# HITRainer/EAVSR

Measured on AMD Instinct MI355X. Metric: SR frames/sec at 4x 7-frame 180x320->720x1280, higher is better.
Workload: dtype f32

## Files before the change

### eavsr_amd/csrc/conv_x6.hip

```cpp
#include "common.h"

#include <mutex>

namespace {

typedef const __attribute__((address_space(1))) void* gptr_t;
typedef __attribute__((address_space(3))) void* lptr_t;
typedef unsigned u32x4 __attribute__((ext_vector_type(4)));
typedef __bf16 bf16x8 __attribute__((ext_vector_type(8)));

constexpr int S_NW = 8, S_TW = 32;
template <int KS, int MT, int NT, int NP = 3> struct C7 {
  static constexpr int PAD = KS / 2, KK = KS * KS;
  static constexpr int KSTEPS = (KK + 1) / 2;
  static constexpr int SLAB = KS == 5 ? 7 : 5;
  static constexpr int NSLAB = (KSTEPS + SLAB - 1) / SLAB;
  static constexpr int TH = S_NW * NT;
  static constexpr int IH = TH + KS - 1;
  static constexpr int IW = S_TW + KS;
  static constexpr int NPIX = IH * IW;
  static constexpr int PLANE_B = NPIX * 16;
  static constexpr int PATCH_B = NP * PLANE_B;
  static constexpr int KS_U4 = NP * MT * 64;
  static constexpr int SLAB_U4 = SLAB * KS_U4;
  static constexpr size_t LDS_BYTES = 2 * (size_t)PATCH_B + 2 * (size_t)SLAB_U4 * 16 + 64 * 4;
  static_assert(NPIX <= 1024, "two patch pixels per thread");
  static_assert(LDS_BYTES <= 160 * 1024, "LDS");
};

struct C7Args {
  const float* x;
  const u32x4* wsplit;
  const float* bias;
  float* out;
  int n, cin, cout, h, w, tiles_x, tiles_y;
  int act;
  float slope;
  int sig_from;
};

__device__ __forceinline__ void s_split2(float a, float b, unsigned& hi, unsigned& mid, unsigned& lo) {
  const unsigned ua = __float_as_uint(a), ub = __float_as_uint(b);
  const float ra = a - __uint_as_float(ua & 0xFFFF0000u), rb = b - __uint_as_float(ub & 0xFFFF0000u);
  const unsigned uma = __float_as_uint(ra), umb = __float_as_uint(rb);
  const float la = ra - __uint_as_float(uma & 0xFFFF0000u), lb = rb - __uint_as_float(umb & 0xFFFF0000u);
  hi = __builtin_amdgcn_perm(ub, ua, 0x07060302u);
  mid = __builtin_amdgcn_perm(umb, uma, 0x07060302u);
  lo = __builtin_amdgcn_perm(__float_as_uint(lb), __float_as_uint(la), 0x07060302u);
}

__device__ __forceinline__ f32x16 s_mfma(const u32x4& a, const u32x4& b, const f32x16& c) {
  return __builtin_amdgcn_mfma_f32_32x32x16_bf16(__builtin_bit_cast(bf16x8, a), __builtin_bit_cast(bf16x8, b), c, 0, 0, 0);
}
typedef _Float16 s_h16x8 __attribute__((ext_vector_type(8)));
__device__ __forceinline__ f32x16 s_mfma_f16(const u32x4& a, const u32x4& b, const f32x16& c) {
  return __builtin_amdgcn_mfma_f32_32x32x16_f16(__builtin_bit_cast(s_h16x8, a), __builtin_bit_cast(s_h16x8, b), c, 0, 0, 0);
}
template <int DT> __device__ __forceinline__ unsigned s_round2(float a, float b) {
  if (DT == 1) return (unsigned)__builtin_bit_cast(unsigned short, (_Float16)a) | ((unsigned)__builtin_bit_cast(unsigned short, (_Float16)b) << 16);
  typedef float f2_ __attribute__((ext_vector_type(2)));
  typedef __bf16 b2_ __attribute__((ext_vector_type(2)));
  return __builtin_bit_cast(unsigned, __builtin_convertvector(f2_{a, b}, b2_));
}

#ifdef EAVSR_C7_STAMPS
__device__ unsigned long long g_c7_stamps[8];
#define C7_STAMP(i)                                                   \
  do {                                                                \
    const unsigned long long t_ = __builtin_amdgcn_s_memtime();       \
    st_acc[i] += t_ - st_last;                                        \
    st_last = t_;                                                     \
  } while (0)
#else
#define C7_STAMP(i) do { } while (0)
#endif

template <int KS, int MT, int NT, int WMT, int NP = 3, int DT = 0, bool PERSIST = false>
__global__ __launch_bounds__(512) void conv_x6_kernel(C7Args a) {
  static_assert((NP == 3 && DT == 0) || (NP == 1 && (DT == 1 || DT == 2)), "three exact bf16 planes, or one rounded fp16 / bf16 plane");
  using K = C7<KS, MT, NT, NP>;
  constexpr int S_NT = NT, S_TH = K::TH, S_NPIX = K::NPIX, S_PLANE_B = K::PLANE_B, S_PATCH_B = K::PATCH_B;
  constexpr int S_PAD = K::PAD, S_IW = K::IW, S_KSTEPS = K::KSTEPS, S_SLAB = K::SLAB, S_NSLAB = K::NSLAB;
#ifdef EAVSR_C7_STAMPS
  unsigned long long st_acc[8] = {0, 0, 0, 0, 0, 0, 0, 0};
  unsigned long long st_last = __builtin_amdgcn_s_memtime();
#endif
  extern __shared__ __attribute__((aligned(16))) unsigned char smem7[];
  unsigned char* s_patch = smem7;
  u32x4* s_w = reinterpret_cast<u32x4*>(smem7 + 2 * S_PATCH_B);
  float* s_bias = reinterpret_cast<float*>(smem7 + 2 * S_PATCH_B + 2 * K::SLAB_U4 * 16);

  const int tid = threadIdx.x;
  const int lane = tid & 63;
  const int wave = __builtin_amdgcn_readfirstlane(tid >> 6);
#if defined(EAVSR_X6_PRIO) && EAVSR_X6_PRIO == 1
  if (wave < 4) __builtin_amdgcn_s_setprio(1);
#elif defined(EAVSR_X6_PRIO) && EAVSR_X6_PRIO == 2
  if (wave >= 4) __builtin_amdgcn_s_setprio(1);
#endif
  const int l31 = lane & 31, kg = lane >> 5;

  const int ntiles = a.tiles_x * a.tiles_y * a.n;
  int tile = PERSIST ? (int)blockIdx.x : eavsr_xcd_remap(blockIdx.x, gridDim.x);
  int bn, y0, x0;
  auto place = [&](int t_, int& bn_, int& y0_, int& x0_) __attribute__((always_inline)) {
    const int tx = t_ % a.tiles_x;
    t_ /= a.tiles_x;
    bn_ = t_ / a.tiles_y;
    y0_ = (t_ - bn_ * a.tiles_y) * S_TH;
    x0_ = tx * S_TW;
  };
  place(tile, bn, y0, x0);
  const int cot = blockIdx.y;
  const int h = a.h, w = a.w;
  const size_t plane = (size_t)h * w;
  const int nch = a.cin >> 3;

  bool pok[2];
  unsigned pgo[2], plo[2];
  int pbn;
  auto aim_patch = [&](int t_) __attribute__((always_inline)) {
    int py0, px0;
    place(t_, pbn, py0, px0);
#pragma unroll
    for (int i = 0; i < 2; ++i) {
      const int p = tid + i * 512;
      const int r = p / S_IW, c = p - r * S_IW;
      const int gy = py0 - S_PAD + r, gx = px0 - S_PAD + c;
      pok[i] = p < S_NPIX && c < S_IW - 1 && gy >= 0 && gy < h && gx >= 0 && gx < w;
      pgo[i] = pok[i] ? (unsigned)(gy * w + gx) : 0u;
      plo[i] = (unsigned)p * 16u;
    }
  };
  aim_patch(tile);
  const bool second = tid + 512 < S_NPIX;
  float pv[2][8];
  auto load_patch = [&](int ch) __attribute__((always_inline)) {
    const float* sp = a.x + ((size_t)pbn * a.cin + (size_t)ch * 8) * plane;
#pragma unroll
    for (int i = 0; i < 2; ++i)
#pragma unroll
      for (int j = 0; j < 8; ++j) pv[i][j] = pok[i] ? sp[(size_t)j * plane + pgo[i]] : 0.f;
  };
  auto store_patch = [&](int stage) __attribute__((always_inline)) {
#pragma unroll
    for (int i = 0; i < 2; ++i) {
      if (i == 0 ? tid >= S_NPIX : !second) break;
      u32x4 pl[NP];
#pragma unroll
      for (int c = 0; c < 4; ++c) {
        if constexpr (NP == 3) {
          unsigned h2, m2, l2;
          s_split2(pv[i][2 * c], pv[i][2 * c + 1], h2, m2, l2);
          pl[0][c] = h2; pl[1][c] = m2; pl[2][c] = l2;
        } else {
          pl[0][c] = s_round2<DT>(pv[i][2 * c], pv[i][2 * c + 1]);
        }
      }
#pragma unroll
      for (int p3 = 0; p3 < NP; ++p3)
        *reinterpret_cast<u32x4*>(s_patch + stage * S_PATCH_B + p3 * S_PLANE_B + plo[i]) = pl[p3];
    }
  };
  const int nslabs = nch * S_NSLAB;
  constexpr int wsplit_n = WMT / MT;
  const int wcot = cot / wsplit_n, wsub = (cot - wcot * wsplit_n) * MT;
  auto issue_slab = [&](int gs, int ch, int si) __attribute__((always_inline)) {
    const int nks = (si + 1) * S_SLAB <= S_KSTEPS ? S_SLAB : S_KSTEPS - si * S_SLAB;
    const int segs = nks * NP * MT;
    const char* wsrc = reinterpret_cast<const char*>(a.wsplit + (((size_t)wcot * nch + ch) * S_KSTEPS + si * S_SLAB) * (K::KS_U4 * wsplit_n));
    u32x4* dst = s_w + (gs & 1) * K::SLAB_U4;
#pragma unroll
    for (int i = 0; i < (S_SLAB * NP * MT + S_NW - 1) / S_NW; ++i) {
      const int seg = i * S_NW + wave;
      if (seg < segs) {
        const int sp = MT == 1 ? seg * WMT + wsub : (seg >> 1) * WMT + wsub + (seg & 1);
        __builtin_amdgcn_global_load_lds((gptr_t)(wsrc + (unsigned)(sp * 64 + lane) * 16u), (lptr_t)(dst + seg * 64), 16, 0, 0);
      }
    }
  };

  f32x16 acc[MT][S_NT];

  const int bbase = ((wave * S_NT) * S_IW + l31) * 16;
  const int b_same = bbase + (kg ? 16 : 0);
  const int b_wrap = bbase + (kg ? (S_IW - (KS - 1)) * 16 : 0);
  const int b_last = kg ? (S_IW - 1) * 16 - ((KS - 1) * S_IW + KS - 1) * 16 : bbase;
  auto read_b = [&](int stage, int s, u32x4 (&b)[S_NT][NP]) __attribute__((always_inline)) {
    const int tap0 = 2 * s, ky = tap0 / KS, kx = tap0 - KS * ky;
    const unsigned char* base = s_patch + stage * S_PATCH_B + ((s == S_KSTEPS - 1 ? b_last : kx == KS - 1 ? b_wrap : b_same) + (ky * S_IW + kx) * 16);
#pragma unroll
    for (int t = 0; t < S_NT; ++t)
#pragma unroll
      for (int p3 = 0; p3 < NP; ++p3) b[t][p3] = *reinterpret_cast<const u32x4*>(base + t * S_IW * 16 + p3 * S_PLANE_B);
  };
  auto read_a = [&](int gs, int sl, u32x4 (&av)[NP][MT]) __attribute__((always_inline)) {
    const u32x4* ws = s_w + (gs & 1) * K::SLAB_U4 + sl * K::KS_U4 + lane;
#pragma unroll
    for (int p3 = 0; p3 < NP; ++p3)
#pragma unroll
      for (int m = 0; m < MT; ++m) av[p3][m] = ws[(p3 * MT + m) * 64];
  };

  issue_slab(0, 0, 0);
  load_patch(0);
  if (tid < 32 * MT) {
    const int co = cot * 32 * MT + tid;
    s_bias[tid] = (a.bias && co < a.cout) ? a.bias[co] : 0.f;
  }
  store_patch(0);
  asm volatile("s_waitcnt vmcnt(0)" ::: "memory");
  __syncthreads();
  auto init_acc = [&]() __attribute__((always_inline)) {
#pragma unroll
    for (int m = 0; m < MT; ++m)
#pragma unroll
      for (int r = 0; r < 16; ++r) {
        const float bv = s_bias[m * 32 + (r & 3) + 8 * (r >> 2) + 4 * kg];
#pragma unroll
        for (int t = 0; t < S_NT; ++t) acc[m][t][r] = bv;
      }
  };
  init_acc();
  if (nslabs > 1) issue_slab(1, S_NSLAB > 1 ? 0 : 1, S_NSLAB > 1 ? 1 : 0);
  u32x4 acur[NP][MT], bcur[S_NT][NP];
  read_a(0, 0, acur);
  read_b(0, 0, bcur);
  C7_STAMP(0);

  for (;;) {
  const bool has_next = PERSIST && tile + (int)gridDim.x < ntiles;
  for (int ch = 0; ch < nch; ++ch) {
    const int pst = ch & 1;
    const bool last_ch = ch + 1 == nch;
    const bool more = !last_ch || has_next;
    if (!last_ch) load_patch(ch + 1);
    else if (has_next) {
      aim_patch(tile + (int)gridDim.x);
      load_patch(0);
    }
#pragma unroll
    for (int ks = 0; ks < S_KSTEPS; ++ks) {
      constexpr int STORE_KS = KS == 7 ? 11 : KS == 5 ? 7 : 3;
      const int si = ks / S_SLAB, sl = ks % S_SLAB;
      const int gs = ch * S_NSLAB + si;
      const bool slab_end = sl == S_SLAB - 1 || ks == S_KSTEPS - 1;
      if (slab_end) {
        C7_STAMP(1);
        asm volatile("s_waitcnt vmcnt(0)" ::: "memory");
        C7_STAMP(2);
        __syncthreads();
        C7_STAMP(3);
        if (gs + 2 < nslabs) issue_slab(gs + 2, ch + (si + 2) / S_NSLAB, (si + 2) % S_NSLAB);
        else if (has_next) issue_slab(gs + 2 - nslabs, (gs + 2 - nslabs) / S_NSLAB, (si + 2) % S_NSLAB);
        C7_STAMP(4);
      }
      if (ks == STORE_KS && more) store_patch(pst ^ 1);
      u32x4 anext[NP][MT], bnext[S_NT][NP];
      const bool last = ks == S_KSTEPS - 1;
      if (!last) {
        read_a(slab_end ? gs + 1 : gs, slab_end ? 0 : sl + 1, anext);
        read_b(pst, ks + 1, bnext);
      } else if (more) {
        read_a(gs + 1, 0, anext);
        read_b(pst ^ 1, 0, bnext);
      }
#pragma unroll
      for (int t = 0; t < S_NT; ++t)
#pragma unroll
        for (int m = 0; m < MT; ++m) {
          f32x16 c_ = acc[m][t];
          if constexpr (NP == 3) {
            c_ = s_mfma(acur[2][m], bcur[t][0], c_);
            c_ = s_mfma(acur[0][m], bcur[t][2], c_);
            c_ = s_mfma(acur[1][m], bcur[t][1], c_);
            c_ = s_mfma(acur[1][m], bcur[t][0], c_);
            c_ = s_mfma(acur[0][m], bcur[t][1], c_);
            c_ = s_mfma(acur[0][m], bcur[t][0], c_);
          } else if constexpr (DT == 1) {
            c_ = s_mfma_f16(acur[0][m], bcur[t][0], c_);
          } else {
            c_ = s_mfma(acur[0][m], bcur[t][0], c_);
          }
          acc[m][t] = c_;
        }
      {
        constexpr int NRD = NP * MT + NP * S_NT, NMF = (NP == 3 ? 6 : 1) * MT * S_NT;
        constexpr int NIL = NRD < NMF ? NRD : NMF;
#pragma unroll
        for (int i = 0; i < NIL; ++i) {
          __builtin_amdgcn_sched_group_barrier(0x008, 1, 0);
          __builtin_amdgcn_sched_group_barrier(0x100, 1, 0);
        }
        if constexpr (NMF > NRD) __builtin_amdgcn_sched_group_barrier(0x008, NMF - NRD, 0);
        if constexpr (NRD > NMF) __builtin_amdgcn_sched_group_barrier(0x100, NRD - NMF, 0);
        __builtin_amdgcn_sched_barrier(0);
      }
      if (!last || more) {
#pragma unroll
        for (int p3 = 0; p3 < NP; ++p3) {
#pragma unroll
          for (int m = 0; m < MT; ++m) acur[p3][m] = anext[p3][m];
#pragma unroll
          for (int t = 0; t < S_NT; ++t) bcur[t][p3] = bnext[t][p3];
        }
      }
    }
  }

  C7_STAMP(1);
  {
  int gx = x0 + l31;
  asm volatile("" : "+v"(gx));
  const bool xok = gx < w;
  const float act_s = a.act == EAVSR_ACT_NONE ? 1.f : a.act == EAVSR_ACT_RELU ? 0.f : a.slope;
  const int co0 = cot * 32 * MT + 4 * kg;
  float* ob = a.out + ((size_t)bn * a.cout + co0) * plane + (size_t)(y0 + wave * S_NT) * w + gx;
  const bool full = cot * 32 * MT + 32 * MT <= a.cout;
#pragma unroll
  for (int m = 0; m < MT; ++m)
#pragma unroll
    for (int r = 0; r < 16; ++r) {
      const int cu = m * 32 + (r & 3) + 8 * (r >> 2);
      const bool cok = full || co0 + cu < a.cout;
      const bool sg = a.sig_from >= 0 && cot * 32 * MT + m * 32 + 8 * (r >> 2) >= a.sig_from;
#pragma unroll
      for (int t = 0; t < S_NT; ++t) {
        float v = acc[m][t][r];
        if (sg) v = eavsr_sigmoid_fast(v);
        else v = eavsr_act(v, act_s);
        if (cok && xok && y0 + wave * S_NT + t < h) ob[(size_t)cu * plane + (size_t)t * w] = v;
      }
    }
  }
  if (!has_next) break;
  tile += (int)gridDim.x;
  place(tile, bn, y0, x0);
  init_acc();
  }
#ifdef EAVSR_C7_STAMPS
  C7_STAMP(5);
  asm volatile("s_waitcnt vmcnt(0)" ::: "memory");
  C7_STAMP(6);
  if (tid == 0)
    for (int i = 0; i < 8; ++i) atomicAdd(&g_c7_stamps[i], st_acc[i]);
#endif
}

__global__ void pack7_kernel(const float* __restrict__ wt, u32x4* __restrict__ p, int cout, int cin, int kk, int mt_n, long total,
                             int np = 3, int dt = 0, int tr = 0) {
  const int ksteps = (kk + 1) / 2;
  const long e = (long)blockIdx.x * blockDim.x + threadIdx.x;
  if (e >= total) return;
  long q = e;
  const int lane = (int)(q % 64); q /= 64;
  const int mt = (int)(q % mt_n); q /= mt_n;
  const int pl = (int)(q % np); q /= np;
  const int s = (int)(q % ksteps); q /= ksteps;
  const int nch = cin / 8;
  const int ch = (int)(q % nch);
  const int cot = (int)(q / nch);
  const int co = cot * 32 * mt_n + mt * 32 + (lane & 31);
  const int tap = 2 * s + (lane >> 5);
  u32x4 o;
#pragma unroll
  for (int c = 0; c < 4; ++c) {
    float v[2];
#pragma unroll
    for (int u = 0; u < 2; ++u) {
      const int ci = ch * 8 + 2 * c + u;
      v[u] = (co < cout && tap < kk) ? (tr ? wt[((size_t)ci * cout + co) * kk + (kk - 1 - tap)] : wt[((size_t)co * cin + ci) * kk + tap]) : 0.f;
    }
    if (np == 3) {
      unsigned h2, m2, l2;
      s_split2(v[0], v[1], h2, m2, l2);
      o[c] = pl == 0 ? h2 : pl == 1 ? m2 : l2;
    } else {
      o[c] = dt == 1 ? s_round2<1>(v[0], v[1]) : s_round2<2>(v[0], v[1]);
    }
  }
  p[e] = o;
}

constexpr int PM_MAX = 48;
struct PackMultiArgs {
  const float* src[PM_MAX];
  u32x4* dst[PM_MAX];
  unsigned long long tr_mask;
};
template <int NP>
__global__ void pack7_multi_kernel(PackMultiArgs a, int cout, int cin, int kk, int mt_n, long total) {
  const int t = blockIdx.y;
  const int tr = (int)((a.tr_mask >> t) & 1ull);
  const float* __restrict__ wt = a.src[t];
  u32x4* __restrict__ p = a.dst[t];
  const int ksteps = (kk + 1) / 2;
  const long e = (long)blockIdx.x * blockDim.x + threadIdx.x;
  if (e >= total) return;
  long q = e;
  const int lane = (int)(q % 64); q /= 64;
  const int mt = (int)(q % mt_n); q /= mt_n;
  const int pl = (int)(q % NP); q /= NP;
  const int s = (int)(q % ksteps); q /= ksteps;
  const int nch = cin / 8;
  const int ch = (int)(q % nch);
  const int cot = (int)(q / nch);
  const int co = cot * 32 * mt_n + mt * 32 + (lane & 31);
  const int tap = 2 * s + (lane >> 5);
  u32x4 o;
#pragma unroll
  for (int c = 0; c < 4; ++c) {
    float v[2];
#pragma unroll
    for (int u = 0; u < 2; ++u) {
      const int ci = ch * 8 + 2 * c + u;
      v[u] = (co < cout && tap < kk) ? (tr ? wt[((size_t)ci * cout + co) * kk + (kk - 1 - tap)] : wt[((size_t)co * cin + ci) * kk + tap]) : 0.f;
    }
    if constexpr (NP == 3) {
      unsigned h2, m2, l2;
      s_split2(v[0], v[1], h2, m2, l2);
      o[c] = pl == 0 ? h2 : pl == 1 ? m2 : l2;
    } else {
      o[c] = s_round2<2>(v[0], v[1]);
    }
  }
  p[e] = o;
}

int mt_of(int cout) { return cout > 32 ? 2 : 1; }

int cu_count() {
  static int cus_pd[eavsr::kMaxDevices] = {};
  static eavsr::PerDeviceOnce once_pd;
  const int dev_ = eavsr::current_device();
  std::call_once(once_pd.flag[dev_], [&] {
    int v = 0;
    if (hipDeviceGetAttribute(&v, hipDeviceAttributeMultiprocessorCount, dev_) == hipSuccess && v > 0) cus_pd[dev_] = v;
  });
  return cus_pd[dev_];
}

int persist_grid(long tiles, int cot_n, int cin) {
  const int slots = cu_count() / cot_n;
  if (slots < 1 || tiles <= slots || (cin >> 3) % 2) return 0;
  const long rounds = (tiles + slots - 1) / slots;
  return (int)((tiles + rounds - 1) / rounds);
}

template <int KS, int MT, int NT, int WMT, int NP = 3, int DT = 0, bool PERSIST = false>
int launch7(const C7Args& a, void* stream, int grid_x = 0) {
  using K = C7<KS, MT, NT, NP>;
  static_assert(!PERSIST || K::NSLAB % 2 == 0, "the slab ring must come round to stage 0 at a tile's start");
  static eavsr::PerDeviceOnce once_pd;
  const int dev_ = eavsr::current_device();
  static hipError_t attr_err_pd[eavsr::kMaxDevices] = {};
  hipError_t& attr_err = attr_err_pd[dev_];
  std::call_once(once_pd.flag[dev_], [&] {
    attr_err = hipFuncSetAttribute(reinterpret_cast<const void*>(&conv_x6_kernel<KS, MT, NT, WMT, NP, DT, PERSIST>),
                                   hipFuncAttributeMaxDynamicSharedMemorySize, (int)K::LDS_BYTES);
  });
  if (attr_err != hipSuccess) {
    eavsr::set_error("conv_f32x6: hipFuncSetAttribute(%zu B of LDS): %s", K::LDS_BYTES, hipGetErrorString(attr_err));
    return (int)attr_err;
  }
  C7Args b = a;
  b.tiles_y = eavsr::cdiv(a.h, K::TH);
  const long blocks = (long)b.tiles_x * b.tiles_y * b.n;
  EAVSR_REQUIRE(blocks < (1L << 31), -1, "conv_f32x6: too many tiles");
  dim3 grid((unsigned)(PERSIST ? grid_x : blocks), eavsr::cdiv(a.cout, 32 * MT));
  hipLaunchKernelGGL((conv_x6_kernel<KS, MT, NT, WMT, NP, DT, PERSIST>), grid, dim3(64 * S_NW), K::LDS_BYTES, eavsr::as_stream(stream), b);
  return eavsr::launch_status("conv_f32x6");
}

template <int KS, int NP = 3, int DT = 0>
int dispatch7(const C7Args& a, void* stream) {
  const long wg2 = (long)a.tiles_x * eavsr::cdiv(a.h, 16) * a.n;
  const long wg1 = (long)a.tiles_x * eavsr::cdiv(a.h, 8) * a.n;
  EAVSR_REQUIRE(wg1 * 2 < (1L << 31), -1, "conv_f32x6: too many tiles");
  if (mt_of(a.cout) == 2) {
    if constexpr (KS == 5 && NP == 3) {
      const int g = wg2 >= 128 ? persist_grid(wg2, eavsr::cdiv(a.cout, 64), a.cin) : 0;
      if (g > 0) return launch7<KS, 2, 2, 2, NP, DT, true>(a, stream, g);
    }
    if (wg2 >= 128) return launch7<KS, 2, 2, 2, NP, DT>(a, stream);
    if (wg1 >= 128) return launch7<KS, 2, 1, 2, NP, DT>(a, stream);
    return launch7<KS, 1, 1, 2, NP, DT>(a, stream);
  }
  if (wg2 >= 128) return launch7<KS, 1, 2, 1, NP, DT>(a, stream);
  return launch7<KS, 1, 1, 1, NP, DT>(a, stream);
}

}

#ifdef EAVSR_C7_STAMPS
extern "C" int eavsr_debug_c7_stamps(unsigned long long* host_out, int reset) {
  hipError_t e = hipMemcpyFromSymbol(host_out, HIP_SYMBOL(g_c7_stamps), sizeof(unsigned long long) * 8);
  if (e != hipSuccess) return (int)e;
  if (reset) {
    unsigned long long z[8] = {0, 0, 0, 0, 0, 0, 0, 0};
    e = hipMemcpyToSymbol(HIP_SYMBOL(g_c7_stamps), z, sizeof(z));
  }
  return (int)e;
}
#endif

extern "C" size_t eavsr_conv_weight_x6_bytes(int32_t ksize, int32_t cout, int32_t cin) {
  if ((ksize != 3 && ksize != 5 && ksize != 7) || cout <= 0 || cin <= 0 || cin % 8) return 0;
  const int mt = mt_of(cout);
  return (size_t)eavsr::cdiv(cout, 32 * mt) * (cin / 8) * ((ksize * ksize + 1) / 2) * 3 * mt * 64 * 16;
}

extern "C" int eavsr_pack_conv_weight_x6(const float* weight, void* packed, int32_t ksize, int32_t cout, int32_t cin, void* stream) {
  EAVSR_REQUIRE(weight && packed, -1, "pack_conv_weight_x6: NULL pointer");
  EAVSR_REQUIRE(ksize == 3 || ksize == 5 || ksize == 7, -2, "pack_conv_weight_x6: kernel size %d (3, 5 and 7 only)", ksize);
  EAVSR_REQUIRE(cout > 0 && cin > 0 && cin % 8 == 0, -1, "pack_conv_weight_x6: cin %d must be a multiple of 8", cin);
  const long total = (long)(eavsr_conv_weight_x6_bytes(ksize, cout, cin) / 16);
  hipLaunchKernelGGL(pack7_kernel, dim3((unsigned)((total + 255) / 256)), dim3(256), 0, eavsr::as_stream(stream), weight,
                     reinterpret_cast<u32x4*>(packed), cout, cin, ksize * ksize, mt_of(cout), total);
  return eavsr::launch_status("pack_conv_weight_x6");
}

extern "C" int eavsr_pack_conv_weight_x6_dgrad(const float* weight, void* packed, int32_t ksize, int32_t cout_w, int32_t cin_w, void* stream) {
  EAVSR_REQUIRE(weight && packed, -1, "pack_conv_weight_x6_dgrad: NULL pointer");
  EAVSR_REQUIRE(ksize == 3 || ksize == 5 || ksize == 7, -2, "pack_conv_weight_x6_dgrad: kernel size %d (3, 5 and 7 only)", ksize);
  EAVSR_REQUIRE(cout_w > 0 && cin_w > 0 && cout_w % 8 == 0, -1, "pack_conv_weight_x6_dgrad: cout %d must be a multiple of 8", cout_w);
  const long total = (long)(eavsr_conv_weight_x6_bytes(ksize, cin_w, cout_w) / 16);
  hipLaunchKernelGGL(pack7_kernel, dim3((unsigned)((total + 255) / 256)), dim3(256), 0, eavsr::as_stream(stream), weight,
                     reinterpret_cast<u32x4*>(packed), cin_w, cout_w, ksize * ksize, mt_of(cin_w), total, 3, 0, 1);
  return eavsr::launch_status("pack_conv_weight_x6_dgrad");
}

extern "C" int eavsr_pack_conv_weight_x6_multi(const float* const* weights, void* const* packed, const int32_t* transposed, int32_t count,
                                               int32_t ksize, int32_t c, void* stream) {
  EAVSR_REQUIRE(count >= 0 && (count == 0 || (weights && packed && transposed)), -1, "pack_conv_weight_x6_multi: NULL pointer");
  EAVSR_REQUIRE(ksize == 3 || ksize == 5 || ksize == 7, -2, "pack_conv_weight_x6_multi: kernel size %d (3, 5 and 7 only)", ksize);
  EAVSR_REQUIRE(c > 0 && c % 8 == 0, -1, "pack_conv_weight_x6_multi: %d channels must be a multiple of 8", c);
  const long total = (long)(eavsr_conv_weight_x6_bytes(ksize, c, c) / 16);
  for (int t0 = 0; t0 < count; t0 += PM_MAX) {
    PackMultiArgs a;
    a.tr_mask = 0ull;
    const int m = count - t0 < PM_MAX ? count - t0 : PM_MAX;
    for (int t = 0; t < PM_MAX; ++t) {
      const int u = t < m ? t0 + t : t0;
      EAVSR_REQUIRE(weights[u] && packed[u], -1, "pack_conv_weight_x6_multi: NULL pointer in entry %d", u);
      a.src[t] = weights[u];
      a.dst[t] = reinterpret_cast<u32x4*>(packed[u]);
      if (t < m && transposed[u]) a.tr_mask |= 1ull << t;
    }
    hipLaunchKernelGGL(pack7_multi_kernel<3>, dim3((unsigned)((total + 255) / 256), (unsigned)m), dim3(256), 0, eavsr::as_stream(stream), a, c,
                       c, ksize * ksize, mt_of(c), total);
  }
  return eavsr::launch_status("pack_conv_weight_x6_multi");
}

extern "C" size_t eavsr_conv_weight_bf16x1_bytes(int32_t ksize, int32_t cout, int32_t cin) {
  return ksize == 3 ? eavsr_conv_weight_x6_bytes(ksize, cout, cin) / 3 : 0;
}

extern "C" int eavsr_pack_conv_weight_bf16x1(const float* weight, void* packed, int32_t ksize, int32_t cout, int32_t cin, void* stream) {
  EAVSR_REQUIRE(weight && packed, -1, "pack_conv_weight_bf16x1: NULL pointer");
  EAVSR_REQUIRE(ksize == 3, -2, "pack_conv_weight_bf16x1: kernel size %d (3 only)", ksize);
  EAVSR_REQUIRE(cout > 0 && cin > 0 && cin % 8 == 0, -1, "pack_conv_weight_bf16x1: cin %d must be a multiple of 8", cin);
  const long total = (long)(eavsr_conv_weight_bf16x1_bytes(ksize, cout, cin) / 16);
  hipLaunchKernelGGL(pack7_kernel, dim3((unsigned)((total + 255) / 256)), dim3(256), 0, eavsr::as_stream(stream), weight,
                     reinterpret_cast<u32x4*>(packed), cout, cin, ksize * ksize, mt_of(cout), total, 1, 2);
  return eavsr::launch_status("pack_conv_weight_bf16x1");
}

extern "C" int eavsr_pack_conv_weight_bf16x1_dgrad(const float* weight, void* packed, int32_t ksize, int32_t cout_w, int32_t cin_w, void* stream) {
  EAVSR_REQUIRE(weight && packed, -1, "pack_conv_weight_bf16x1_dgrad: NULL pointer");
  EAVSR_REQUIRE(ksize == 3, -2, "pack_conv_weight_bf16x1_dgrad: kernel size %d (3 only)", ksize);
  EAVSR_REQUIRE(cout_w > 0 && cin_w > 0 && cout_w % 8 == 0, -1, "pack_conv_weight_bf16x1_dgrad: cout %d must be a multiple of 8", cout_w);
  const long total = (long)(eavsr_conv_weight_bf16x1_bytes(ksize, cin_w, cout_w) / 16);
  hipLaunchKernelGGL(pack7_kernel, dim3((unsigned)((total + 255) / 256)), dim3(256), 0, eavsr::as_stream(stream), weight,
                     reinterpret_cast<u32x4*>(packed), cin_w, cout_w, ksize * ksize, mt_of(cin_w), total, 1, 2, 1);
  return eavsr::launch_status("pack_conv_weight_bf16x1_dgrad");
}

extern "C" int eavsr_pack_conv_weight_bf16x1_multi(const float* const* weights, void* const* packed, const int32_t* transposed,
                                                   int32_t count, int32_t ksize, int32_t c, void* stream) {
  EAVSR_REQUIRE(count >= 0 && (count == 0 || (weights && packed && transposed)), -1, "pack_conv_weight_bf16x1_multi: NULL pointer");
  EAVSR_REQUIRE(ksize == 3, -2, "pack_conv_weight_bf16x1_multi: kernel size %d (3 only)", ksize);
  EAVSR_REQUIRE(c > 0 && c % 8 == 0, -1, "pack_conv_weight_bf16x1_multi: %d channels must be a multiple of 8", c);
  const long total = (long)(eavsr_conv_weight_bf16x1_bytes(ksize, c, c) / 16);
  for (int t0 = 0; t0 < count; t0 += PM_MAX) {
    PackMultiArgs a;
    a.tr_mask = 0ull;
    const int m = count - t0 < PM_MAX ? count - t0 : PM_MAX;
    for (int t = 0; t < PM_MAX; ++t) {
      const int u = t < m ? t0 + t : t0;
      EAVSR_REQUIRE(weights[u] && packed[u], -1, "pack_conv_weight_bf16x1_multi: NULL pointer in entry %d", u);
      a.src[t] = weights[u];
      a.dst[t] = reinterpret_cast<u32x4*>(packed[u]);
      if (t < m && transposed[u]) a.tr_mask |= 1ull << t;
    }
    hipLaunchKernelGGL(pack7_multi_kernel<1>, dim3((unsigned)((total + 255) / 256), (unsigned)m), dim3(256), 0, eavsr::as_stream(stream), a, c,
                       c, ksize * ksize, mt_of(c), total);
  }
  return eavsr::launch_status("pack_conv_weight_bf16x1_multi");
}

extern "C" int32_t eavsr_conv_f32x6_tiles_per_workgroup(int32_t n, int32_t cin, int32_t cout, int32_t h, int32_t w, int32_t ksize) {
  if (ksize != 5 || n <= 0 || cin <= 0 || cout <= 0 || h <= 0 || w <= 0 || mt_of(cout) != 2) return 1;
  const long wg2 = (long)eavsr::cdiv(w, S_TW) * eavsr::cdiv(h, 16) * n;
  const int g = wg2 >= 128 ? persist_grid(wg2, eavsr::cdiv(cout, 64), cin) : 0;
  return g > 0 ? (int32_t)((wg2 + g - 1) / g) : 1;
}

extern "C" int eavsr_conv_f32x6(const float* x, const void* weight_x6, const float* bias, float* out, int32_t n, int32_t cin,
                                int32_t cout, int32_t h, int32_t w, int32_t ksize, int32_t act, float slope, int32_t sigmoid_from,
                                void* stream) {
#ifndef EAVSR_X6_KS3
  EAVSR_REQUIRE(ksize == 5 || ksize == 7, -2, "conv_f32x6: kernel size %d (5 and 7 only; 3x3 is eavsr_conv2d_f32 / eavsr_conv3x3_wino4_f32 / eavsr_conv3x3_f32x6s)", ksize);
#endif
  EAVSR_REQUIRE(n >= 0 && cin > 0 && cout > 0 && h > 0 && w > 0, -1, "conv_f32x6: bad dims");
  if (n == 0) return 0;
  EAVSR_REQUIRE(x && weight_x6 && out, -1, "conv_f32x6: NULL pointer");
  EAVSR_REQUIRE(cin % 8 == 0, -2, "conv_f32x6: cin %d must be a multiple of 8 (use eavsr_conv2d_f32)", cin);
  EAVSR_REQUIRE(act >= 0 && act <= 2, -1, "conv_f32x6: act %d", act);
  EAVSR_REQUIRE(act != EAVSR_ACT_LRELU || (slope >= 0.f && slope <= 1.f), -2,
                "conv_f32x6: leaky-ReLU slope %g outside [0, 1] (the epilogue evaluates max(v, slope v))", (double)slope);
  EAVSR_REQUIRE((long)h * w < (1L << 31), -1, "conv_f32x6: image plane too large for 32-bit pixel offsets");
  EAVSR_REQUIRE(sigmoid_from < 0 || (sigmoid_from % 8 == 0 && sigmoid_from < cout), -2,
                "conv_f32x6: sigmoid_from %d (a multiple of 8 below cout, or -1)", sigmoid_from);
  C7Args a;
  a.x = x; a.wsplit = reinterpret_cast<const u32x4*>(weight_x6); a.bias = bias; a.out = out;
  a.n = n; a.cin = cin; a.cout = cout; a.h = h; a.w = w;
  a.tiles_x = eavsr::cdiv(w, S_TW);
  a.tiles_y = 0;
  a.act = act; a.slope = slope; a.sig_from = sigmoid_from < 0 ? -1 : sigmoid_from;
#ifdef EAVSR_X6_KS3
  if (ksize == 3) return dispatch7<3>(a, stream);
#endif
  return ksize == 7 ? dispatch7<7>(a, stream) : dispatch7<5>(a, stream);
}

extern "C" size_t eavsr_conv_weight_h16x1_bytes(int32_t ksize, int32_t cout, int32_t cin) {
  return eavsr_conv_weight_x6_bytes(ksize, cout, cin) / 3;
}

extern "C" int eavsr_pack_conv_weight_h16x1(const float* weight, void* packed, int32_t ksize, int32_t cout, int32_t cin, int32_t dtype,
                                            void* stream) {
  EAVSR_REQUIRE(weight && packed, -1, "pack_conv_weight_h16x1: NULL pointer");
  EAVSR_REQUIRE(ksize == 7, -2, "pack_conv_weight_h16x1: kernel size %d (7 only)", ksize);
  EAVSR_REQUIRE(dtype == 1 || dtype == 2, -1, "pack_conv_weight_h16x1: dtype %d (1 = f16, 2 = bf16)", dtype);
  EAVSR_REQUIRE(cout > 0 && cin > 0 && cin % 8 == 0, -1, "pack_conv_weight_h16x1: cin %d must be a multiple of 8", cin);
  const long total = (long)(eavsr_conv_weight_h16x1_bytes(ksize, cout, cin) / 16);
  hipLaunchKernelGGL(pack7_kernel, dim3((unsigned)((total + 255) / 256)), dim3(256), 0, eavsr::as_stream(stream), weight,
                     reinterpret_cast<u32x4*>(packed), cout, cin, ksize * ksize, mt_of(cout), total, 1, dtype);
  return eavsr::launch_status("pack_conv_weight_h16x1");
}

extern "C" int eavsr_conv_h16x1(const float* x, const void* weight_h16x1, const float* bias, float* out, int32_t n, int32_t cin,
                                int32_t cout, int32_t h, int32_t w, int32_t ksize, int32_t act, float slope, int32_t dtype, void* stream) {
  EAVSR_REQUIRE(ksize == 7, -2, "conv_h16x1: kernel size %d (7 only)", ksize);
  EAVSR_REQUIRE(dtype == 1 || dtype == 2, -1, "conv_h16x1: dtype %d (1 = f16, 2 = bf16)", dtype);
  EAVSR_REQUIRE(n >= 0 && cin > 0 && cout > 0 && h > 0 && w > 0, -1, "conv_h16x1: bad dims");
  if (n == 0) return 0;
  EAVSR_REQUIRE(x && weight_h16x1 && out, -1, "conv_h16x1: NULL pointer");
  EAVSR_REQUIRE(cin % 8 == 0, -2, "conv_h16x1: cin %d must be a multiple of 8", cin);
  EAVSR_REQUIRE(act >= 0 && act <= 2, -1, "conv_h16x1: act %d", act);
  EAVSR_REQUIRE(act != EAVSR_ACT_LRELU || (slope >= 0.f && slope <= 1.f), -2, "conv_h16x1: leaky-ReLU slope %g outside [0, 1]", (double)slope);
  EAVSR_REQUIRE((long)h * w < (1L << 31), -1, "conv_h16x1: image plane too large for 32-bit pixel offsets");
  C7Args a;
  a.x = x; a.wsplit = reinterpret_cast<const u32x4*>(weight_h16x1); a.bias = bias; a.out = out;
  a.n = n; a.cin = cin; a.cout = cout; a.h = h; a.w = w;
  a.tiles_x = eavsr::cdiv(w, S_TW);
  a.tiles_y = 0;
  a.act = act; a.slope = slope; a.sig_from = -1;
  return dtype == 1 ? dispatch7<7, 1, 1>(a, stream) : dispatch7<7, 1, 2>(a, stream);
}
```

Measured before the change: 138.9.

## Extend persistent conv_x6 to 7x7 and MT=1, interleave weight DMA with MFMAs

Result: no change. 139.1 (median of 4 runs) (+0.1%).

```diff
diff --git a/eavsr_amd/csrc/conv_x6.hip b/eavsr_amd/csrc/conv_x6.hip
--- a/eavsr_amd/csrc/conv_x6.hip
+++ b/eavsr_amd/csrc/conv_x6.hip
@@ -23,6 +23,7 @@
   static constexpr int PATCH_B = NP * PLANE_B;
   static constexpr int KS_U4 = NP * MT * 64;
   static constexpr int SLAB_U4 = SLAB * KS_U4;
+  static constexpr int SLAB_PIECES = (SLAB * NP * MT + S_NW - 1) / S_NW;
   static constexpr size_t LDS_BYTES = 2 * (size_t)PATCH_B + 2 * (size_t)SLAB_U4 * 16 + 64 * 4;
   static_assert(NPIX <= 1024, "two patch pixels per thread");
   static_assert(LDS_BYTES <= 160 * 1024, "LDS");
@@ -64,15 +65,18 @@
 }
 
 #ifdef EAVSR_C7_STAMPS
-__device__ unsigned long long g_c7_stamps[8];
+constexpr int C7_NSTAMP = 12;
+__device__ unsigned long long g_c7_stamps[C7_NSTAMP];
 #define C7_STAMP(i)                                                   \
   do {                                                                \
     const unsigned long long t_ = __builtin_amdgcn_s_memtime();       \
     st_acc[i] += t_ - st_last;                                        \
     st_last = t_;                                                     \
   } while (0)
+#define C7_WAIT_OPERANDS() asm volatile("s_waitcnt lgkmcnt(0)" ::: "memory")
 #else
 #define C7_STAMP(i) do { } while (0)
+#define C7_WAIT_OPERANDS() do { } while (0)
 #endif
 
 template <int KS, int MT, int NT, int WMT, int NP = 3, int DT = 0, bool PERSIST = false>
@@ -82,8 +86,10 @@
   constexpr int S_NT = NT, S_TH = K::TH, S_NPIX = K::NPIX, S_PLANE_B = K::PLANE_B, S_PATCH_B = K::PATCH_B;
   constexpr int S_PAD = K::PAD, S_IW = K::IW, S_KSTEPS = K::KSTEPS, S_SLAB = K::SLAB, S_NSLAB = K::NSLAB;
 #ifdef EAVSR_C7_STAMPS
-  unsigned long long st_acc[8] = {0, 0, 0, 0, 0, 0, 0, 0};
+  unsigned long long st_acc[C7_NSTAMP] = {};
+  const unsigned long long st_rt0 = __builtin_amdgcn_s_memrealtime();
   unsigned long long st_last = __builtin_amdgcn_s_memtime();
+  C7_STAMP(10);
 #endif
   extern __shared__ __attribute__((aligned(16))) unsigned char smem7[];
   unsigned char* s_patch = smem7;
@@ -165,18 +171,19 @@
   const int nslabs = nch * S_NSLAB;
   constexpr int wsplit_n = WMT / MT;
   const int wcot = cot / wsplit_n, wsub = (cot - wcot * wsplit_n) * MT;
-  auto issue_slab = [&](int gs, int ch, int si) __attribute__((always_inline)) {
+  const unsigned lane16 = (unsigned)lane * 16u;
+  auto issue_slab = [&](int stage, int ch, int si) __attribute__((always_inline)) {
     const int nks = (si + 1) * S_SLAB <= S_KSTEPS ? S_SLAB : S_KSTEPS - si * S_SLAB;
     const int segs = nks * NP * MT;
     const char* wsrc = reinterpret_cast<const char*>(a.wsplit + (((size_t)wcot * nch + ch) * S_KSTEPS + si * S_SLAB) * (K::KS_U4 * wsplit_n));
-    u32x4* dst = s_w + (gs & 1) * K::SLAB_U4;
-#pragma unroll
-    for (int i = 0; i < (S_SLAB * NP * MT + S_NW - 1) / S_NW; ++i) {
-      const int seg = i * S_NW + wave;
-      if (seg < segs) {
-        const int sp = MT == 1 ? seg * WMT + wsub : (seg >> 1) * WMT + wsub + (seg & 1);
-        __builtin_amdgcn_global_load_lds((gptr_t)(wsrc + (unsigned)(sp * 64 + lane) * 16u), (lptr_t)(dst + seg * 64), 16, 0, 0);
-      }
+    u32x4* dst = s_w + stage * K::SLAB_U4;
+#pragma unroll
+    for (int i = 0; i < K::SLAB_PIECES; ++i) {
+      if (i * S_NW >= segs) break;
+      int seg = i * S_NW + wave;
+      seg = seg < segs ? seg : segs - 1;
+      const int sp = MT == 1 ? seg * WMT + wsub : (seg >> 1) * WMT + wsub + (seg & 1);
+      __builtin_amdgcn_global_load_lds((gptr_t)(wsrc + (size_t)sp * 1024 + lane16), (lptr_t)(dst + seg * 64), 16, 0, 0);
     }
   };
 
@@ -239,6 +246,7 @@
       aim_patch(tile + (int)gridDim.x);
       load_patch(0);
     }
+    C7_STAMP(6);
 #pragma unroll
     for (int ks = 0; ks < S_KSTEPS; ++ks) {
       constexpr int STORE_KS = KS == 7 ? 11 : KS == 5 ? 7 : 3;
@@ -246,24 +254,29 @@
       const int gs = ch * S_NSLAB + si;
       const bool slab_end = sl == S_SLAB - 1 || ks == S_KSTEPS - 1;
       if (slab_end) {
-        C7_STAMP(1);
         asm volatile("s_waitcnt vmcnt(0)" ::: "memory");
-        C7_STAMP(2);
+        C7_STAMP(3);
         __syncthreads();
-        C7_STAMP(3);
-        if (gs + 2 < nslabs) issue_slab(gs + 2, ch + (si + 2) / S_NSLAB, (si + 2) % S_NSLAB);
-        else if (has_next) issue_slab(gs + 2 - nslabs, (gs + 2 - nslabs) / S_NSLAB, (si + 2) % S_NSLAB);
         C7_STAMP(4);
       }
-      if (ks == STORE_KS && more) store_patch(pst ^ 1);
+      if (ks == STORE_KS && more) {
+        store_patch(pst ^ 1);
+        C7_STAMP(7);
+      }
       u32x4 anext[NP][MT], bnext[S_NT][NP];
       const bool last = ks == S_KSTEPS - 1;
       if (!last) {
         read_a(slab_end ? gs + 1 : gs, slab_end ? 0 : sl + 1, anext);
         read_b(pst, ks + 1, bnext);
-      } else if (more) {
+      } else {
         read_a(gs + 1, 0, anext);
         read_b(pst ^ 1, 0, bnext);
+      }
+      if (slab_end) {
+        int c2 = ch + (si + 2) / S_NSLAB;
+        c2 = c2 < nch ? c2 : c2 - nch;
+        if constexpr (S_NSLAB == 1) c2 = c2 < nch ? c2 : c2 - nch;
+        issue_slab(gs & 1, c2, (si + 2) % S_NSLAB);
       }
 #pragma unroll
       for (int t = 0; t < S_NT; ++t)
@@ -287,28 +300,39 @@
       {
         constexpr int NRD = NP * MT + NP * S_NT, NMF = (NP == 3 ? 6 : 1) * MT * S_NT;
         constexpr int NIL = NRD < NMF ? NRD : NMF;
+        constexpr int NDMA = K::SLAB_PIECES < NMF - NIL ? K::SLAB_PIECES : NMF - NIL;
 #pragma unroll
         for (int i = 0; i < NIL; ++i) {
           __builtin_amdgcn_sched_group_barrier(0x008, 1, 0);
           __builtin_amdgcn_sched_group_barrier(0x100, 1, 0);
         }
-        if constexpr (NMF > NRD) __builtin_amdgcn_sched_group_barrier(0x008, NMF - NRD, 0);
         if constexpr (NRD > NMF) __builtin_amdgcn_sched_group_barrier(0x100, NRD - NMF, 0);
+        if (slab_end) {
+#pragma unroll
+          for (int i = 0; i < NDMA; ++i) {
+            __builtin_amdgcn_sched_group_barrier(0x008, 1, 0);
+            __builtin_amdgcn_sched_group_barrier(0x010, 1, 0);
+          }
+          if constexpr (NMF - NIL > NDMA) __builtin_amdgcn_sched_group_barrier(0x008, NMF - NIL - NDMA, 0);
+          if constexpr (K::SLAB_PIECES > NDMA) __builtin_amdgcn_sched_group_barrier(0x010, K::SLAB_PIECES - NDMA, 0);
+        } else if constexpr (NMF > NRD) {
+          __builtin_amdgcn_sched_group_barrier(0x008, NMF - NRD, 0);
+        }
         __builtin_amdgcn_sched_barrier(0);
       }
-      if (!last || more) {
-#pragma unroll
-        for (int p3 = 0; p3 < NP; ++p3) {
-#pragma unroll
-          for (int m = 0; m < MT; ++m) acur[p3][m] = anext[p3][m];
-#pragma unroll
-          for (int t = 0; t < S_NT; ++t) bcur[t][p3] = bnext[t][p3];
-        }
-      }
-    }
-  }
-
-  C7_STAMP(1);
+      C7_STAMP(1);
+      C7_WAIT_OPERANDS();
+      C7_STAMP(2);
+#pragma unroll
+      for (int p3 = 0; p3 < NP; ++p3) {
+#pragma unroll
+        for (int m = 0; m < MT; ++m) acur[p3][m] = anext[p3][m];
+#pragma unroll
+        for (int t = 0; t < S_NT; ++t) bcur[t][p3] = bnext[t][p3];
+      }
+    }
+  }
+
   {
   int gx = x0 + l31;
   asm volatile("" : "+v"(gx));
@@ -333,17 +357,18 @@
       }
     }
   }
+  C7_STAMP(8);
   if (!has_next) break;
   tile += (int)gridDim.x;
   place(tile, bn, y0, x0);
   init_acc();
   }
 #ifdef EAVSR_C7_STAMPS
-  C7_STAMP(5);
   asm volatile("s_waitcnt vmcnt(0)" ::: "memory");
-  C7_STAMP(6);
+  C7_STAMP(9);
+  st_acc[11] = __builtin_amdgcn_s_memrealtime() - st_rt0;
   if (tid == 0)
-    for (int i = 0; i < 8; ++i) atomicAdd(&g_c7_stamps[i], st_acc[i]);
+    for (int i = 0; i < C7_NSTAMP; ++i) atomicAdd(&g_c7_stamps[i], st_acc[i]);
 #endif
 }
 
@@ -447,10 +472,14 @@
   return (int)((tiles + rounds - 1) / rounds);
 }
 
+int persist_grid7(int n, int cin, int cout, int h, int w) {
+  const long wg2 = (long)eavsr::cdiv(w, S_TW) * eavsr::cdiv(h, 16) * n;
+  return wg2 >= 128 ? persist_grid(wg2, eavsr::cdiv(cout, 32 * mt_of(cout)), cin) : 0;
+}
+
 template <int KS, int MT, int NT, int WMT, int NP = 3, int DT = 0, bool PERSIST = false>
 int launch7(const C7Args& a, void* stream, int grid_x = 0) {
   using K = C7<KS, MT, NT, NP>;
-  static_assert(!PERSIST || K::NSLAB % 2 == 0, "the slab ring must come round to stage 0 at a tile's start");
   static eavsr::PerDeviceOnce once_pd;
   const int dev_ = eavsr::current_device();
   static hipError_t attr_err_pd[eavsr::kMaxDevices] = {};
@@ -478,14 +507,18 @@
   const long wg1 = (long)a.tiles_x * eavsr::cdiv(a.h, 8) * a.n;
   EAVSR_REQUIRE(wg1 * 2 < (1L << 31), -1, "conv_f32x6: too many tiles");
   if (mt_of(a.cout) == 2) {
-    if constexpr (KS == 5 && NP == 3) {
-      const int g = wg2 >= 128 ? persist_grid(wg2, eavsr::cdiv(a.cout, 64), a.cin) : 0;
+    if constexpr (NP == 3) {
+      const int g = persist_grid7(a.n, a.cin, a.cout, a.h, a.w);
       if (g > 0) return launch7<KS, 2, 2, 2, NP, DT, true>(a, stream, g);
     }
     if (wg2 >= 128) return launch7<KS, 2, 2, 2, NP, DT>(a, stream);
     if (wg1 >= 128) return launch7<KS, 2, 1, 2, NP, DT>(a, stream);
     return launch7<KS, 1, 1, 2, NP, DT>(a, stream);
   }
+  if constexpr (NP == 3) {
+    const int g = persist_grid7(a.n, a.cin, a.cout, a.h, a.w);
+    if (g > 0) return launch7<KS, 1, 2, 1, NP, DT, true>(a, stream, g);
+  }
   if (wg2 >= 128) return launch7<KS, 1, 2, 1, NP, DT>(a, stream);
   return launch7<KS, 1, 1, 1, NP, DT>(a, stream);
 }
@@ -494,10 +527,10 @@
 
 #ifdef EAVSR_C7_STAMPS
 extern "C" int eavsr_debug_c7_stamps(unsigned long long* host_out, int reset) {
-  hipError_t e = hipMemcpyFromSymbol(host_out, HIP_SYMBOL(g_c7_stamps), sizeof(unsigned long long) * 8);
+  hipError_t e = hipMemcpyFromSymbol(host_out, HIP_SYMBOL(g_c7_stamps), sizeof(unsigned long long) * C7_NSTAMP);
   if (e != hipSuccess) return (int)e;
   if (reset) {
-    unsigned long long z[8] = {0, 0, 0, 0, 0, 0, 0, 0};
+    unsigned long long z[C7_NSTAMP] = {};
     e = hipMemcpyToSymbol(HIP_SYMBOL(g_c7_stamps), z, sizeof(z));
   }
   return (int)e;
@@ -601,9 +634,9 @@
 }
 
 extern "C" int32_t eavsr_conv_f32x6_tiles_per_workgroup(int32_t n, int32_t cin, int32_t cout, int32_t h, int32_t w, int32_t ksize) {
-  if (ksize != 5 || n <= 0 || cin <= 0 || cout <= 0 || h <= 0 || w <= 0 || mt_of(cout) != 2) return 1;
+  if ((ksize != 5 && ksize != 7) || n <= 0 || cin <= 0 || cout <= 0 || h <= 0 || w <= 0 || cin % 8) return 1;
   const long wg2 = (long)eavsr::cdiv(w, S_TW) * eavsr::cdiv(h, 16) * n;
-  const int g = wg2 >= 128 ? persist_grid(wg2, eavsr::cdiv(cout, 64), cin) : 0;
+  const int g = persist_grid7(n, cin, cout, h, w);
   return g > 0 ? (int32_t)((wg2 + g - 1) / g) : 1;
 }
 
```
